# pengpeng-yu/FastPCC

Hardware: NVIDIA B200
Metric: encode+decode Mpts/s (higher is better)
Workload: dtype int8

## Files before the change

fastpcc_b200/csrc/igemm_tc.cu:

```cuda
#include <cuda.h>
#include <cuda_bf16.h>
#include <cuda_fp16.h>

#include <map>
#include <mutex>
#include <tuple>

#include "common.cuh"
#include "epi_nt.cuh"

namespace fpcc {

constexpr int TC_M = 128;
constexpr int TC_KB = 128;
constexpr int TC_MAX_KVOL = 32;

__device__ __forceinline__ uint32_t smem_u32(const void *p) { return (uint32_t)__cvta_generic_to_shared(p); }

__device__ __forceinline__ void mbar_init(uint64_t *bar, uint32_t count) {
    asm volatile("mbarrier.init.shared::cta.b64 [%0], %1;" ::"r"(smem_u32(bar)), "r"(count));
}
__device__ __forceinline__ void mbar_arrive(uint64_t *bar) {
    asm volatile("mbarrier.arrive.shared::cta.b64 _, [%0];" ::"r"(smem_u32(bar)) : "memory");
}
// ... 32 lines not shown
    asm volatile("mov.u32 %0, %%cluster_ctarank;" : "=r"(r));
    return r;
}
__device__ __forceinline__ uint32_t mapa_u32(uint32_t local_smem_addr, uint32_t rank) {
    uint32_t a;
    asm volatile("mapa.shared::cluster.u32 %0, %1, %2;" : "=r"(a) : "r"(local_smem_addr), "r"(rank));
    return a;
}
__device__ __forceinline__ void cluster_sync_all() {
    asm volatile("barrier.cluster.arrive.release.aligned;" ::: "memory");
    asm volatile("barrier.cluster.wait.acquire.aligned;" ::: "memory");
}
__device__ __forceinline__ void mbar_wait_cluster(uint64_t *bar, uint32_t parity) {
    asm volatile(
        "{\n\t"
        ".reg .pred p;\n\t"
        "WAITC_LOOP:\n\t"
        "mbarrier.try_wait.parity.acquire.cluster.shared::cta.b64 p, [%0], %1, %2;\n\t"
        "@p bra.uni WAITC_DONE;\n\t"
        "bra.uni WAITC_LOOP;\n\t"
        "WAITC_DONE:\n\t"
        "}" ::"r"(smem_u32(bar)), "r"(parity), "r"(0x989680u) : "memory");
}
__device__ __forceinline__ void tma_load_2d_mc(uint32_t dst, const CUtensorMap *map, uint64_t *bar, int c0, int c1, uint16_t cta_mask) {
    asm volatile(
        "cp.async.bulk.tensor.2d.shared::cluster.global.mbarrier::complete_tx::bytes.multicast::cluster [%0], [%1, {%3, %4}], [%2], %5;"
        ::"r"(dst), "l"(map), "r"(smem_u32(bar)), "r"(c0), "r"(c1), "h"(cta_mask) : "memory");
}
__device__ __forceinline__ void umma_commit_mc(uint64_t *bar, uint16_t cta_mask) {
    asm volatile("tcgen05.commit.cta_group::1.mbarrier::arrive::one.shared::cluster.multicast::cluster.b64 [%0], %1;"
                 ::"r"(smem_u32(bar)), "h"(cta_mask) : "memory");
}
__device__ __forceinline__ void cp_async16(uint32_t dst, const void *src, uint32_t src_bytes) {
    asm volatile("cp.async.cg.shared.global [%0], [%1], 16, %2;" ::"r"(dst), "l"(src), "r"(src_bytes) : "memory");
}
__device__ __forceinline__ void cp_async_commit() { asm volatile("cp.async.commit_group;" ::: "memory"); }
template <int N>
__device__ __forceinline__ void cp_async_wait() { asm volatile("cp.async.wait_group %0;" ::"n"(N) : "memory"); }
__device__ __forceinline__ void fence_proxy_async() { asm volatile("fence.proxy.async.shared::cta;" ::: "memory"); }
__device__ __forceinline__ void tc_fence_before() { asm volatile("tcgen05.fence::before_thread_sync;" ::: "memory"); }
__device__ __forceinline__ void tc_fence_after() { asm volatile("tcgen05.fence::after_thread_sync;" ::: "memory"); }

__device__ __forceinline__ void tma_load_2d(uint32_t dst, const CUtensorMap *map, uint64_t *bar, int c0, int c1) {
    asm volatile(
        "cp.async.bulk.tensor.2d.shared::cluster.global.mbarrier::complete_tx::bytes [%0], [%1, {%3, %4}], [%2];"
        ::"r"(dst), "l"(map), "r"(smem_u32(bar)), "r"(c0), "r"(c1) : "memory");
}

__device__ __forceinline__ uint64_t umma_desc_sw128(uint32_t smem_addr) {
    uint64_t d = 0;
    d |= (uint64_t)((smem_addr & 0x3FFFFu) >> 4);
    d |= (uint64_t)(1024u >> 4) << 32;
    d |= (uint64_t)1 << 46;
    d |= (uint64_t)2 << 61;
    return d;
}
__device__ __forceinline__ uint32_t umma_idesc_i8(int n) {
    return (2u << 4) | (1u << 7) | (1u << 10) | ((uint32_t)(n >> 3) << 17) | ((uint32_t)(TC_M >> 4) << 24);
}
__device__ __forceinline__ uint32_t umma_idesc_f16(int n, int bf16) {
    return (1u << 4) | ((uint32_t)bf16 << 7) | ((uint32_t)bf16 << 10) | ((uint32_t)(n >> 3) << 17) | ((uint32_t)(TC_M >> 4) << 24);
}
__device__ __forceinline__ void umma_f16(uint32_t tmem_d, uint64_t adesc, uint64_t bdesc, uint32_t idesc, uint32_t accumulate) {
    asm volatile(
        "{\n\t"
        ".reg .pred p;\n\t"
        "setp.ne.b32 p, %4, 0;\n\t"
        "tcgen05.mma.cta_group::1.kind::f16 [%0], %1, %2, %3, p;\n\t"
        "}" ::"r"(tmem_d), "l"(adesc), "l"(bdesc), "r"(idesc), "r"(accumulate) : "memory");
}
__device__ __forceinline__ void umma_i8(uint32_t tmem_d, uint64_t adesc, uint64_t bdesc, uint32_t idesc, uint32_t accumulate) {
    asm volatile(
        "{\n\t"
        ".reg .pred p;\n\t"
        "setp.ne.b32 p, %4, 0;\n\t"
        "tcgen05.mma.cta_group::1.kind::i8 [%0], %1, %2, %3, p;\n\t"
        "}" ::"r"(tmem_d), "l"(adesc), "l"(bdesc), "r"(idesc), "r"(accumulate) : "memory");
}
__device__ __forceinline__ void umma_commit(uint64_t *bar) {
    asm volatile("tcgen05.commit.cta_group::1.mbarrier::arrive::one.shared::cluster.b64 [%0];" ::"r"(smem_u32(bar)) : "memory");
}
__device__ __forceinline__ void tmem_ld16(uint32_t taddr, uint32_t (&r)[16]) {
    asm volatile(
        "tcgen05.ld.sync.aligned.32x32b.x16.b32 "
        "{%0, %1, %2, %3, %4, %5, %6, %7, %8, %9, %10, %11, %12, %13, %14, %15}, [%16];"
        : "=r"(r[0]), "=r"(r[1]), "=r"(r[2]), "=r"(r[3]), "=r"(r[4]), "=r"(r[5]), "=r"(r[6]), "=r"(r[7]), "=r"(r[8]),
          "=r"(r[9]), "=r"(r[10]), "=r"(r[11]), "=r"(r[12]), "=r"(r[13]), "=r"(r[14]), "=r"(r[15])
        : "r"(taddr));
    asm volatile("tcgen05.wait::ld.sync.aligned;" ::: "memory");
}

#ifdef FPCC_TC_TRACE
__device__ unsigned long long g_trace[4096][8];
__device__ __forceinline__ void trace_stamp(int j, int slot) {
    if (blockIdx.x == 0 && j < 4096) {
        unsigned long long t;
        asm volatile("mov.u64 %0, %%globaltimer;" : "=l"(t));
        g_trace[j][slot] = t;
    }
}
#define TRACE(j, slot) trace_stamp((j), (slot))
#else
#define TRACE(j, slot)
#endif

struct TcArgs {
    const int8_t *A;
    int K;
    int N;
    int n_tile;
    int tmem_cols;
    const int32_t *nbr;
    int64_t ld;
    int n_out, kvol;
    const int32_t *row_perm;
    const int32_t *in_idx, *out_idx, *offsets;
    int n_groups, n_pairs, bias_per_group;
};

constexpr int EC = 16;

template <int WORDS>
__device__ __forceinline__ void store_words(char *optr, const uint32_t (&w)[WORDS], int nbytes) {
#pragma unroll
    for (int t = 0; t < WORDS / 4; ++t)
        if (t * 16 < nbytes) reinterpret_cast<uint4 *>(optr)[t] = make_uint4(w[4 * t], w[4 * t + 1], w[4 * t + 2], w[4 * t + 3]);
// ... 698 lines not shown
                if (fe.out_type == 0) ((__half *)optr)[q] = __float2half_rn(o[q]);
                else if (fe.out_type == 1) ((__nv_bfloat16 *)optr)[q] = __float2bfloat16_rn(o[q]);
                else ((float *)optr)[q] = o[q];
            }
        }
    }
}

constexpr int EPI_WARPS_CONV = 12, EPI_WARPS_PAIRS = 16;
#ifndef FPCC_PAIRS_PRODUCER_WARPS
#define FPCC_PAIRS_PRODUCER_WARPS 4
#endif
template <int MODE>
constexpr int prod_warps() { return MODE == 1 ? FPCC_PAIRS_PRODUCER_WARPS : 4; }
static_assert(FPCC_PAIRS_PRODUCER_WARPS == 4 || FPCC_PAIRS_PRODUCER_WARPS == 2, "producer warps: 2 or 4");

struct PMeta {
    uint32_t kmask;
    int32_t group, begin, end;
};

template <int STAGES>
struct PSmem {
    static size_t bytes(int n_tile, int rows_k) {
        return 1024 + (size_t)STAGES * (TC_M * TC_KB + (size_t)n_tile * TC_KB) + 2 * (size_t)rows_k * TC_M * 4 +
               (size_t)n_tile * 20 + 512;
    }
};

__device__ __forceinline__ void pairs_tile_lookup(const TcArgs &a, int tile_m, PMeta *m) {
    int g = 0, begin = tile_m * TC_M, end = a.n_pairs;
    if (a.offsets) {
        int t = tile_m;
        begin = end = -1;
        for (g = 0; g < a.n_groups; ++g) {
            int lo = a.offsets[g], hi = a.offsets[g + 1];
            int nt = (hi - lo + TC_M - 1) / TC_M;
            if (t < nt) { begin = lo + t * TC_M; end = hi; break; }
            t -= nt;
        }
    }
    m->group = g < a.n_groups ? g : a.n_groups - 1; m->begin = begin; m->end = end;
}

enum { OK_I8 = 0, OK_I16 = 1, OK_I32 = 2, OK_POST2 = 3 };

template <int MODE, int STAGES, int KIND, int EW, int OUTK, bool CL2>
__global__ void __launch_bounds__((EW + prod_warps<MODE>() + 2) * 32, 1) igemm_tc_persistent(TcArgs a, const __grid_constant__ CUtensorMap tmap_w,
                                                                    EpiParams ep, FEpi fe, void *__restrict__ out, int tiles_m,
                                                                    int tiles_n) {
    constexpr int PW = prod_warps<MODE>(), PT = PW * 32;
    constexpr int P_EPI_WARPS = EW, P_PROD_WARP0 = EW, P_TMA_WARP = EW + PW, P_MMA_WARP = EW + PW + 1, P_THREADS = (EW + PW + 2) * 32;
    extern __shared__ uint8_t smem_raw[];
    uint8_t *smem = (uint8_t *)(((uintptr_t)smem_raw + 1023) & ~(uintptr_t)1023);
    const int b_bytes = a.n_tile * TC_KB;
    constexpr int a_bytes = TC_M * TC_KB;
    uint8_t *sA = smem;
    uint8_t *sB = smem + STAGES * a_bytes;
    const int rows_k = MODE == 0 ? a.kvol : 2;
    int32_t *rows_s = (int32_t *)(sB + (size_t)STAGES * b_bytes);
    int4 *chan4_s = (int4 *)(rows_s + 2 * rows_k * TC_M);
    int2 *chan_s = (int2 *)chan4_s;
    int32_t *thr_s = (int32_t *)(chan4_s + a.n_tile);
    uint64_t *bars = (uint64_t *)(thr_s + a.n_tile);
    uint64_t *full = bars, *empty = bars + STAGES;
    uint64_t *meta_full = bars + 2 * STAGES, *tmem_full = meta_full + 2, *tmem_empty = tmem_full + 2;
    uint64_t *xchg = tmem_empty + 2;
    uint64_t *meta_empty = xchg + 2;
    PMeta *meta = (PMeta *)(meta_empty + 2);
    uint32_t *tmem_ptr = (uint32_t *)(meta + 2);
    uint32_t *lean_off = tmem_ptr + 1;
    uint32_t *peer_kmask = lean_off + 1;
    uint32_t *nt_flags = peer_kmask + 2;
    const uint32_t cl_rank = CL2 ? cluster_ctarank() : 0u;
    const int p0 = CL2 ? (int)(blockIdx.x >> 1) : (int)blockIdx.x;
    const int p_step = CL2 ? (int)(gridDim.x >> 1) : (int)gridDim.x;

    const int tid = threadIdx.x, warp = tid >> 5, lane = tid & 31;
    const int n_chunks = (a.K + TC_KB - 1) / TC_KB;
    const int total_tiles = tiles_m * tiles_n;
    const int p_end = CL2 ? (total_tiles + 1) / 2 : total_tiles;
#define FPCC_TILE_OF(p) (CL2 ? 2 * (p) + (int)cl_rank : (p))

    if (warp == P_MMA_WARP && lane == 0) {
        for (int s = 0; s < STAGES; ++s) {
            mbar_init(&full[s], PT + 1);
            mbar_init(&empty[s], CL2 ? 2 : 1);
        }
        for (int b = 0; b < 2; ++b) {
            mbar_init(&meta_full[b], PT);
            mbar_init(&tmem_full[b], 1);
            mbar_init(&tmem_empty[b], P_EPI_WARPS);
            mbar_init(&xchg[b], 1);
            mbar_init(&meta_empty[b], P_EPI_WARPS + 2);
        }
        asm volatile("fence.mbarrier_init.release.cluster;" ::: "memory");
    }
    if (warp == P_TMA_WARP && lane == 0) asm volatile("prefetch.tensormap [%0];" ::"l"(&tmap_w) : "memory");
    if (warp == P_MMA_WARP) {
        asm volatile("tcgen05.alloc.cta_group::1.sync.aligned.shared::cta.b32 [%0], %1;" ::"r"(smem_u32(tmem_ptr)), "r"((uint32_t)(2 * a.tmem_cols)) : "memory");
        asm volatile("tcgen05.relinquish_alloc_permit.cta_group::1.sync.aligned;" ::: "memory");
    }
    const bool chan_static = tiles_n == 1 && !(MODE == 1 && a.bias_per_group);
    const int64_t zp_all = KIND == 0 ? ep.zp[0] : 0;
    int64_t vmax = 0;
    const int sgn_mode = KIND == 0 ? lean_mode(ep, zp_all, (int64_t)a.K * (MODE == 0 ? a.kvol : 1), ep.row_bias_bound, &vmax) : SGN_NONE;
    if (tid >= 32 && tid < 48) nt_flags[tid - 32] = 0u;
    if (tid == 0) {
        *lean_off = sgn_mode != SGN_NONE ? 0u : 1u;
        thr_s[0] = (1 << 24) - 1; thr_s[1] = 0;
        if (KIND == 0 && ep.post_mul) {
            const Post2 p2 = load_post2(ep);
            int64_t t2 = 0;
            if (p2.mul) { const int64_t nz = -p2.zp, m = (int64_t)p2.mul; t2 = nz >= 0 ? (nz + m - 1) / m : -((-nz) / m); }
            const int64_t c02 = p2.zp + (p2.shift > 0 ? (int64_t)1 << (p2.shift - 1) : 0);
            thr_s[4] = (int32_t)p2.mul;
            thr_s[5] = (int32_t)(t2 > 2147483647ll ? 2147483647ll : (t2 < -2147483648ll ? -2147483648ll : t2));
            thr_s[6] = p2.slope; thr_s[7] = p2.shift >= 32 ? p2.shift - 32 : 0;
            thr_s[8] = (int32_t)(uint32_t)c02; thr_s[9] = (int32_t)(uint32_t)((uint64_t)c02 >> 32);
            thr_s[10] = (p2.shift >= 32 && !tie_possible(p2.mul, p2.zp, p2.shift, (int64_t)1 << 31)) ? 1 : 0;
        }
    }
    __syncthreads();
    const bool nt_on = FPCC_NT_SMEM && KIND == 0 && OUTK == OK_I8 && sgn_mode != SGN_NONE;
    const int64_t abound = (int64_t)a.K * (MODE == 0 ? a.kvol : 1) * 16384 + (ep.row_bias ? (int64_t)ep.row_bias_bound : 0);
    if (chan_static)
        for (int cb = warp * 32; cb < a.n_tile; cb += P_THREADS) {
            const int c = cb + lane;
            const bool valid = c < a.n_tile;
            if (KIND == 0) {
                const int32_t b = c < a.N && ep.bias ? ep.bias[c] : 0;
                const uint32_t mu = c < a.N ? ep.mul[ep.mul_is_scalar ? 0 : c] : 0u;
                bool ok = true;
                if (valid) {
                    ok = stage_channel(b, mu, zp_all, ep.shift, ep.out_type, vmax, &chan4_s[c]);
                    if (!ok && sgn_mode != SGN_NONE) atomicOr(lean_off, 1u);
                }
                stage_nt_chunks(nt_on, valid, ok, c, b, mu, zp_all, ep.shift, abound, nt_flags);
            } else if (valid) {
                chan_s[c] = make_int2(c < a.N && fe.bias ? __float_as_int(fe.bias[c]) : 0, 0);
            }
        }
    tc_fence_before();
    __syncthreads();
    tc_fence_after();
    if (CL2) cluster_sync_all();
    const uint32_t tmem_base = *tmem_ptr;

    if (warp >= P_PROD_WARP0 && warp < P_PROD_WARP0 + PW) {
        const int r = tid - P_PROD_WARP0 * 32;
        int it = 0;
        int j = 0;
        constexpr int PRE = 27;
        int32_t nv[PRE];
        const bool pre = MODE == 0 && a.kvol <= PRE;
        auto fetch = [&](int t) {
            const int m = (t / tiles_n) * TC_M + r;
            const bool ok = t < total_tiles && m < a.n_out;
#pragma unroll
            for (int u = 0; u < PRE; ++u) nv[u] = (ok && u < a.kvol) ? __ldg(&a.nbr[(int64_t)u * a.ld + m]) : 0;
        };
        if (pre) fetch(FPCC_TILE_OF(p0));
        for (int p = p0; p < p_end; p += p_step, ++j) {
            const int tile = FPCC_TILE_OF(p);
            const int slot = j & 1;
            const int tile_m = tile / tiles_n;
            int32_t *rows = rows_s + slot * rows_k * TC_M;
            if (r == 0) TRACE(j, 0);
            mbar_wait(&meta_empty[slot], ((j >> 1) & 1) ^ 1);
// ... 19 lines not shown
                    }
                }
                mine = __reduce_or_sync(0xffffffffu, mine);
                if (lane == 0 && mine) atomicOr(&meta[slot].kmask, mine);
            } else {
                if (r == 0) { pairs_tile_lookup(a, tile_m, &meta[slot]); }
                asm volatile("bar.sync 1, %0;" ::"n"(PT) : "memory");
#if FPCC_PAIRS_PRODUCER_WARPS == 4
                const int p = meta[slot].begin + r;
                const bool ok = meta[slot].begin >= 0 && p < meta[slot].end;
                rows[r] = ok ? (a.in_idx ? __ldg(&a.in_idx[p]) : p) : -1;
                rows[TC_M + r] = ok ? (a.out_idx ? __ldg(&a.out_idx[p]) : p) : -1;
#else
#pragma unroll
                for (int rr = r; rr < TC_M; rr += PT) {
                    const int p = meta[slot].begin + rr;
                    const bool ok = meta[slot].begin >= 0 && p < meta[slot].end;
                    rows[rr] = ok ? (a.in_idx ? __ldg(&a.in_idx[p]) : p) : -1;
                    rows[TC_M + rr] = ok ? (a.out_idx ? __ldg(&a.out_idx[p]) : p) : -1;
                }
#endif
                if (r == 0) meta[slot].kmask = meta[slot].begin >= 0 && meta[slot].begin < meta[slot].end ? 1u : 0u;
            }
            if (CL2) {
                asm volatile("bar.sync 1, %0;" ::"n"(PT) : "memory");
                if (r == 0) {
                    const uint32_t own = *(volatile uint32_t *)&meta[slot].kmask;
                    const uint32_t peer = cl_rank ^ 1u;
                    asm volatile("st.shared::cluster.u32 [%0], %1;" ::"r"(mapa_u32(smem_u32(&peer_kmask[slot]), peer)), "r"(own) : "memory");
                    asm volatile("mbarrier.arrive.release.cluster.shared::cluster.b64 _, [%0];" ::"r"(mapa_u32(smem_u32(&xchg[slot]), peer)) : "memory");
                    mbar_wait_cluster(&xchg[slot], (j >> 1) & 1);
                    meta[slot].kmask = own | *(volatile uint32_t *)&peer_kmask[slot];
                }
            }
            __threadfence_block();
            mbar_arrive(&meta_full[slot]);
            mbar_wait(&meta_full[slot], (j >> 1) & 1);
            uint32_t rem = meta[slot].kmask;
            const int total = __popc(rem) * n_chunks;
            int k = 0, kc = n_chunks - 1;
            if (r == 0) TRACE(j, 2);
            for (int i = 0; i < total; ++i, ++it) {
                if (++kc == n_chunks) { kc = 0; k = __ffs(rem) - 1; rem &= rem - 1; }
                const int stage = it % STAGES;
                mbar_wait(&empty[stage], ((it / STAGES) & 1) ^ 1);
#if FPCC_PAIRS_PRODUCER_WARPS == 4
                const int base = (r & ~31) + (lane >> 3) * 8;
// ... 36 lines not shown
                }
#endif
                asm volatile("cp.async.mbarrier.arrive.noinc.shared::cta.b64 [%0];" ::"r"(smem_u32(&full[stage])) : "memory");
            }
        }
    } else if (warp == P_TMA_WARP) {
        if (lane == 0) {
            int it = 0, j = 0;
            for (int p = p0; p < p_end; p += p_step, ++j) {
                const int tile = FPCC_TILE_OF(p);
                const int slot = j & 1;
                const int n0 = (tile % tiles_n) * a.n_tile;
                mbar_wait(&meta_full[slot], (j >> 1) & 1);
                uint32_t rem = meta[slot].kmask;
                const int total = __popc(rem) * n_chunks;
                const int group = MODE == 1 ? meta[slot].group : 0;
                mbar_arrive(&meta_empty[slot]);
                int k = 0, kc = n_chunks - 1;
                for (int i = 0; i < total; ++i, ++it) {
                    if (++kc == n_chunks) { kc = 0; k = __ffs(rem) - 1; rem &= rem - 1; }
                    const int stage = it % STAGES;
                    mbar_wait(&empty[stage], ((it / STAGES) & 1) ^ 1);
                    mbar_expect_tx(&full[stage], (uint32_t)b_bytes);
                    const int wrow = (MODE == 0 ? k : group) * a.N + n0;
                    if (CL2) {
                        const int half = a.n_tile >> 1;
                        tma_load_2d_mc(smem_u32(sB + (size_t)stage * b_bytes + (size_t)cl_rank * half * TC_KB), &tmap_w, &full[stage],
                                       kc * TC_KB, wrow + (int)cl_rank * half, (uint16_t)3);
                    } else {
                        tma_load_2d(smem_u32(sB + (size_t)stage * b_bytes), &tmap_w, &full[stage], kc * TC_KB, wrow);
                    }
                }
            }
        }
    } else if (warp == P_MMA_WARP) {
        if (lane == 0) {
            const uint32_t idesc = KIND == 0 ? umma_idesc_i8(a.n_tile) : umma_idesc_f16(a.n_tile, KIND == 2);
            int it = 0, j = 0;
            for (int p = p0; p < p_end; p += p_step, ++j) {
                const int slot = j & 1;
                mbar_wait(&meta_full[slot], (j >> 1) & 1);
                const int total = __popc(meta[slot].kmask) * n_chunks;
                mbar_arrive(&meta_empty[slot]);
                mbar_wait(&tmem_empty[slot], ((j >> 1) & 1) ^ 1);
                tc_fence_after();
                const uint32_t tacc = tmem_base + (uint32_t)(slot * a.tmem_cols);
                for (int i = 0; i < total; ++i, ++it) {
                    const int stage = it % STAGES;
                    mbar_wait(&full[stage], (it / STAGES) & 1);
                    if (i == 0) TRACE(j, 3);
                    fence_proxy_async();
                    tc_fence_after();
                    const uint64_t ad = umma_desc_sw128(smem_u32(sA + stage * a_bytes));
                    const uint64_t bd = umma_desc_sw128(smem_u32(sB + (size_t)stage * b_bytes));
                    {
#pragma unroll
                        for (int q = 0; q < TC_KB / 32; ++q) {
                            if (KIND == 0) umma_i8(tacc, ad + 2 * q, bd + 2 * q, idesc, (uint32_t)(i > 0 || q > 0));
                            else umma_f16(tacc, ad + 2 * q, bd + 2 * q, idesc, (uint32_t)(i > 0 || q > 0));
                        }
                    }
                    if (CL2) umma_commit_mc(&empty[stage], (uint16_t)3);
                    else umma_commit(&empty[stage]);
                }
                TRACE(j, 4);
                if (total > 0) umma_commit(&tmem_full[slot]);
                else mbar_arrive(&tmem_full[slot]);
            }
        }
    } else if (warp < P_EPI_WARPS) {
        const int quarter = warp & 3, group = warp >> 2;
        const int r = quarter * 32 + lane;
        const bool has_slope = KIND == 0 && ep.slope != nullptr, has_post = KIND == 0 && ep.post_slope != nullptr;
        const int32_t slope = has_slope ? ep.slope[0] : 0, post = has_post ? ep.post_slope[0] : 0;
        const int64_t zp = KIND == 0 ? ep.zp[0] : 0;
        const int shift = ep.shift;
        const int cols_grp = (((a.n_tile + P_EPI_WARPS / 4 - 1) / (P_EPI_WARPS / 4) + EC - 1) / EC) * EC;
        const int c_begin = min(a.n_tile, group * cols_grp), c_end = min(a.n_tile, c_begin + cols_grp);
        const bool out_al = ((uintptr_t)out & 15) == 0 && (ep.out_ld & 15) == 0;
        LeanU lu;
        {
            const int64_t c0v = zp + (shift > 0 ? (int64_t)1 << (shift - 1) : 0);
            lu.slope = slope; lu.post = post; lu.shift = shift; { const uint32_t ka = smem_u32(thr_s); int32_t k_lo, k_hi; asm volatile("ld.shared.v2.s32 {%0, %1}, [%2];" : "=r"(k_lo), "=r"(k_hi) : "r"(ka)); lu.k24 = pack64((uint32_t)k_lo, (uint32_t)k_hi); }
            lu.c0_lo = (uint32_t)c0v; lu.c0_hi = (uint32_t)((uint64_t)c0v >> 32);
            lu.ovf_add = shift > 0 && shift <= 31 ? 1u << (shift - 1) : 0u;
            lu.ovf_lim = shift <= 31 ? (1u << shift) - 1u : 0xffffffffu;
        }
        lu.post2_addr = smem_u32(thr_s + 4);
        lu.nt_addr = smem_u32(nt_flags);
        const bool post2_on = KIND == 0 && OUTK == OK_POST2;
// ... 133 lines not shown
                EpiCtx cx;
                cx.chan4 = chan4_s + c0;
                cx.slope = slope; cx.post = post; cx.zp = zp; cx.shift = shift;
                cx.half = shift > 0 ? (int64_t)1 << (shift - 1) : 0; cx.sgn = shift > 0;
                cx.row_bias = ep.row_bias ? ep.row_bias + (int64_t)__ldg(&ep.row_idx[m]) * a.N + nb : nullptr;
                cx.residual = ep.residual ? ep.residual + m * a.N + nb : nullptr;
                cx.has_post = has_post;
                cx.nvalid = min(EC, a.N - nb);
                void *optr = (ep.out_type == FPCC_OUT_I8 || post2_on) ? (void *)((char *)out + m * (ep.out_ld > 0 ? (int64_t)ep.out_ld : (int64_t)a.N) + nb)
                                                                      : (void *)((char *)out + (m * a.N + nb) * (ep.out_type == FPCC_OUT_I16 ? 2 : 4));
                const bool vec = out_al && (a.N & 15) == 0;
                const bool rb = ep.row_bias != nullptr;
                Post2 p2;
                p2.on = false; p2.dual = false;
                if (post2_on || (OUTK == OK_I32 && ep.aux_out)) p2 = load_post2(ep);
                cx.aux = p2.dual ? ep.aux_out + m * a.N + nb : nullptr;
                if (OUTK == OK_I8) epi_dispatch<FPCC_OUT_I8>(acc, cx, optr, vec, has_slope, rb, p2);
                else if (OUTK == OK_I32 || OUTK == OK_POST2) epi_dispatch<FPCC_OUT_I32>(acc, cx, optr, vec, has_slope, rb, p2);
                else epi_dispatch<FPCC_OUT_I16>(acc, cx, optr, vec, has_slope, rb, p2);
            }
            tc_fence_before();
            __syncwarp();
            if (tid == 0) TRACE(j, 6);
            if (lane == 0) mbar_arrive(&tmem_empty[slot]);
        }
    }
    tc_fence_before();
    __syncthreads();
    if (CL2) cluster_sync_all();
    if (warp == P_MMA_WARP) {
        asm volatile("tcgen05.dealloc.cta_group::1.sync.aligned.b32 %0, %1;" ::"r"(tmem_base), "r"((uint32_t)(2 * a.tmem_cols)) : "memory");
    }
#undef FPCC_TILE_OF
}

__global__ void __launch_bounds__(128, 1) mma_i8_peak_kernel(int iters, int n) {
    extern __shared__ uint8_t smem_raw[];
    uint8_t *smem = (uint8_t *)(((uintptr_t)smem_raw + 1023) & ~(uintptr_t)1023);
    __shared__ uint64_t done;
    __shared__ uint32_t tmem_ptr;
    const int warp = threadIdx.x >> 5, lane = threadIdx.x & 31;
    for (int i = threadIdx.x; i < (TC_M * TC_KB + 256 * TC_KB) / 4; i += blockDim.x) ((uint32_t *)smem)[i] = 0x01010101u;
    if (threadIdx.x == 0) {
        mbar_init(&done, 1);
        asm volatile("fence.mbarrier_init.release.cluster;" ::: "memory");
    }
    if (warp == 0) {
        asm volatile("tcgen05.alloc.cta_group::1.sync.aligned.shared::cta.b32 [%0], %1;" ::"r"(smem_u32(&tmem_ptr)), "r"(256u) : "memory");
        asm volatile("tcgen05.relinquish_alloc_permit.cta_group::1.sync.aligned;" ::: "memory");
    }
    fence_proxy_async();
    tc_fence_before();
    __syncthreads();
    tc_fence_after();
    const uint32_t tmem_base = tmem_ptr;
// ... 56 lines not shown
    CUresult r = fn(&m, CU_TENSOR_MAP_DATA_TYPE_UINT8, 2, (void *)w, dims, strides, box, estr, CU_TENSOR_MAP_INTERLEAVE_NONE,
                    CU_TENSOR_MAP_SWIZZLE_128B, CU_TENSOR_MAP_L2_PROMOTION_L2_256B, CU_TENSOR_MAP_FLOAT_OOB_FILL_NONE);
    FPCC_REQUIRE(r == CUDA_SUCCESS, "cuTensorMapEncodeTiled failed with CUresult %d (rows %lld, K %d, box %d)", (int)r, (long long)rows, K, box_rows);
    if (cache.size() > 4096) cache.clear();
    cache[key] = m;
    *out = m;
    return FPCC_OK;
}

static bool tc_shape_ok(const void *A, const void *W, int K, int N) {
    return K >= 32 && K % 16 == 0 && N >= 16 && (((uintptr_t)A | (uintptr_t)W) & 15) == 0;
}

static int pick_tile(int N, int *n_tile, int *tmem_cols) {
    int nt = N >= 256 ? 256 : ((N + 15) / 16) * 16;
    int cols = 32;
    while (cols < nt) cols <<= 1;
    *n_tile = nt;
    *tmem_cols = cols;
    return (N + nt - 1) / nt;
}

constexpr size_t TC_SMEM_MAX = 227 * 1024;
template <int MODE, int STAGES, int KIND, int OUTK>
static int launch_outk(const TcArgs &a, const CUtensorMap &tmap, const EpiParams &ep, const FEpi &fe, void *out, int tiles_m,
                       int n_blocks_n, int grid, size_t smem, bool cl2, cudaStream_t s) {
#ifndef FPCC_CONV2_EW
#define FPCC_CONV2_EW 8
#endif
#ifndef FPCC_LIN32_EW
#define FPCC_LIN32_EW 8
#endif
#ifndef FPCC_LINP2_EW
#define FPCC_LINP2_EW 8
#endif
#ifndef FPCC_CONV1_EW
#define FPCC_CONV1_EW EPI_WARPS_CONV
#endif
#ifndef FPCC_LIN8_EW
#define FPCC_LIN8_EW EPI_WARPS_PAIRS
#endif
    constexpr int EW = KIND != 0 ? (MODE == 0 ? EPI_WARPS_CONV : EPI_WARPS_PAIRS)
                       : MODE == 0 ? ((OUTK == OK_I32 || OUTK == OK_POST2) ? FPCC_CONV2_EW : FPCC_CONV1_EW)
                                   : (OUTK == OK_I32 ? FPCC_LIN32_EW : (OUTK == OK_POST2 ? FPCC_LINP2_EW : FPCC_LIN8_EW));
    constexpr int OK = KIND == 0 ? OUTK : OK_I8;
    constexpr int THREADS = (EW + prod_warps<MODE>() + 2) * 32;
    if (MODE == 0 && KIND == 0 && cl2) {
        auto kern = igemm_tc_persistent<MODE, STAGES, KIND, EW, OK, (MODE == 0 && KIND == 0)>;
        static bool configured = false;
        if (!configured) {
            FPCC_CUDA(cudaFuncSetAttribute(kern, cudaFuncAttributeMaxDynamicSharedMemorySize, (int)TC_SMEM_MAX));
            configured = true;
        }
        cudaLaunchConfig_t cfg = {};
        cfg.gridDim = dim3((unsigned)grid); cfg.blockDim = dim3(THREADS); cfg.dynamicSmemBytes = smem; cfg.stream = s;
        cudaLaunchAttribute attr[1];
        attr[0].id = cudaLaunchAttributeClusterDimension;
        attr[0].val.clusterDim.x = 2; attr[0].val.clusterDim.y = 1; attr[0].val.clusterDim.z = 1;
        cfg.attrs = attr; cfg.numAttrs = 1;
        FPCC_CUDA(cudaLaunchKernelEx(&cfg, kern, a, tmap, ep, fe, out, tiles_m, n_blocks_n));
        return FPCC_OK;
    }
    auto kern = igemm_tc_persistent<MODE, STAGES, KIND, EW, OK, false>;
    static bool configured = false;
    if (!configured) {
        FPCC_CUDA(cudaFuncSetAttribute(kern, cudaFuncAttributeMaxDynamicSharedMemorySize, (int)TC_SMEM_MAX));
        configured = true;
    }
    kern<<<grid, THREADS, smem, s>>>(a, tmap, ep, fe, out, tiles_m, n_blocks_n);
    FPCC_LAUNCH_CHECK();
    return FPCC_OK;
}

template <int MODE, int STAGES, int KIND>
static int launch_stages(const TcArgs &a, const CUtensorMap &tmap, const EpiParams &ep, const FEpi &fe, void *out, int tiles_m,
                         int n_blocks_n, int grid, int rows_k, bool cl2, cudaStream_t s) {
    size_t smem = PSmem<STAGES>::bytes(a.n_tile, rows_k);
    FPCC_REQUIRE(smem <= TC_SMEM_MAX, "igemm_tc: %zu bytes of shared memory exceed the 227 KB limit", smem);
    if (KIND != 0) return launch_outk<MODE, STAGES, KIND, OK_I8>(a, tmap, ep, fe, out, tiles_m, n_blocks_n, grid, smem, cl2, s);
    if (ep.post_mul && !ep.aux_out) return launch_outk<MODE, STAGES, KIND, OK_POST2>(a, tmap, ep, fe, out, tiles_m, n_blocks_n, grid, smem, cl2, s);
    if (ep.out_type == FPCC_OUT_I8) return launch_outk<MODE, STAGES, KIND, OK_I8>(a, tmap, ep, fe, out, tiles_m, n_blocks_n, grid, smem, cl2, s);
    if (ep.out_type == FPCC_OUT_I32) return launch_outk<MODE, STAGES, KIND, OK_I32>(a, tmap, ep, fe, out, tiles_m, n_blocks_n, grid, smem, cl2, s);
    return launch_outk<MODE, STAGES, KIND, OK_I16>(a, tmap, ep, fe, out, tiles_m, n_blocks_n, grid, smem, cl2, s);
}

static int g_cl2_mode = -1;
static bool cl2_enabled() {
    if (g_cl2_mode < 0) {
        const char *e = getenv("FPCC_CL2");
        g_cl2_mode = (e && e[0] == '1') ? 1 : 0;
    }
    return g_cl2_mode == 1;
}

template <int MODE, int KIND>
static int launch_tc(TcArgs &a, const void *W, int64_t w_rows, int tiles_m, const EpiParams &ep, const FEpi &fe, void *out,
                     cudaStream_t s) {
    int n_blocks_n = pick_tile(a.N, &a.n_tile, &a.tmem_cols);
    const int rows_k = MODE == 0 ? a.kvol : 2;
    int total = tiles_m * n_blocks_n;
    int sms = g_sm_budget > 0 && g_sm_budget < sm_count() ? g_sm_budget : sm_count();
    const bool cl2 = MODE == 0 && KIND == 0 && n_blocks_n == 1 && (a.n_tile % 16) == 0 && total >= 4 && sms >= 2 && cl2_enabled();
    CUtensorMap tmap;
    int rc = weight_tensor_map((const int8_t *)W, w_rows, a.K, cl2 ? a.n_tile / 2 : a.n_tile, &tmap);
    if (rc) return rc;
    int grid = total < sms ? total : sms;
    if (cl2) {
        const int pairs = (total + 1) / 2, clusters = sms / 2;
        grid = 2 * (pairs < clusters ? pairs : clusters);
    }
    static const bool force3 = [] { const char *e = getenv("FPCC_STAGES"); return e && e[0] == '3'; }();
    if (!force3 && PSmem<4>::bytes(a.n_tile, rows_k) <= TC_SMEM_MAX)
        return launch_stages<MODE, 4, KIND>(a, tmap, ep, fe, out, tiles_m, n_blocks_n, grid, rows_k, cl2, s);
    return launch_stages<MODE, 3, KIND>(a, tmap, ep, fe, out, tiles_m, n_blocks_n, grid, rows_k, cl2, s);
}

int launch_conv_tc(const int8_t *feats, int n_in, int c_in, const int8_t *weight, int kvol, int c_out, const int32_t *nbr,
                   int64_t ld, int n_out, const int32_t *row_perm, const EpiParams &ep, void *out, cudaStream_t s) {
    (void)n_in;
    if (!tc_shape_ok(feats, weight, c_in, c_out) || kvol > TC_MAX_KVOL) return FPCC_ERR_UNSUPPORTED;
    TcArgs a = {};
    a.A = feats; a.K = c_in; a.N = c_out;
    a.nbr = nbr; a.ld = ld; a.n_out = n_out; a.kvol = kvol; a.row_perm = row_perm;
    FEpi fe = {};
    return launch_tc<0, 0>(a, weight, (int64_t)kvol * c_out, ceil_div(n_out, TC_M), ep, fe, out, s);
}

int launch_pairs_tc(const PairArgs &p, const EpiParams &ep, void *out, int max_tiles, cudaStream_t s) {
    (void)max_tiles;
    if (p.raw != 0 || !tc_shape_ok(p.A, p.W, p.K, p.N)) return FPCC_ERR_UNSUPPORTED;
    TcArgs a = {};
    a.A = p.A; a.K = p.K; a.N = p.N;
    a.in_idx = p.in_idx; a.out_idx = p.out_idx; a.offsets = p.offsets;
    a.n_groups = p.n_groups; a.n_pairs = p.n_pairs; a.bias_per_group = p.bias_per_group;
    int tiles = ceil_div(p.n_pairs, TC_M) + (p.offsets ? p.n_groups : 0);
    FEpi fe = {};
    return launch_tc<1, 0>(a, p.W, (int64_t)p.n_groups * p.N, tiles, ep, fe, out, s);
// ... 259 lines not shown
    cudaStream_t s = (cudaStream_t)stream;
    size_t smem = 1024 + TC_M * TC_KB + 256 * TC_KB;
    FPCC_CUDA(cudaFuncSetAttribute(mma_i8_peak_kernel, cudaFuncAttributeMaxDynamicSharedMemorySize, (int)smem));
    cudaEvent_t e0, e1;
    FPCC_CUDA(cudaEventCreate(&e0));
    FPCC_CUDA(cudaEventCreate(&e1));
    int sms = sm_count();
    mma_i8_peak_kernel<<<sms, 128, smem, s>>>(iters / 8 + 1, n);
    FPCC_CUDA(cudaEventRecord(e0, s));
    mma_i8_peak_kernel<<<sms, 128, smem, s>>>(iters, n);
    FPCC_CUDA(cudaEventRecord(e1, s));
    FPCC_CUDA(cudaEventSynchronize(e1));
    float ms = 0;
    FPCC_CUDA(cudaEventElapsedTime(&ms, e0, e1));
    cudaEventDestroy(e0);
    cudaEventDestroy(e1);
    *tops_out = 2.0 * TC_M * n * 32.0 * 4.0 * iters * sms / (ms * 1e-3) / 1e12;
    return FPCC_OK;
}

#ifdef FPCC_TC_TRACE
extern "C" int fpcc_trace_read(unsigned long long *host, int n) {
    FPCC_CUDA(cudaDeviceSynchronize());
    FPCC_CUDA(cudaMemcpyFromSymbol(host, fpcc::g_trace, sizeof(unsigned long long) * 8 * (size_t)n));
    return FPCC_OK;
}
#endif

extern "C" int fpcc_gemm_engine(int k, int n, int kvol, int has_zp_comp) {
    return fpcc::tc_enabled() && !has_zp_comp && k >= 32 && k % 16 == 0 && n >= 16 && kvol <= fpcc::TC_MAX_KVOL;
}

extern "C" int fpcc_set_sm_budget(int sms) {
    fpcc::g_sm_budget = sms > 0 ? sms : 0;
    return FPCC_OK;
}

extern "C" int fpcc_set_tc_mode(int mode) {
    fpcc::g_tc_mode = mode ? 1 : 0;
    return FPCC_OK;
}
```

Baseline: 24.90.

## Use 2-CTA paired tcgen05 MMA for sparse conv tiles by default

Replaces the opt-in 2-CTA cluster mode, which multicast weights via TMA, with a true cta_group::2 UMMA path. Each CTA loads half of the weight tile and the leader issues M=256 MMAs spanning both CTAs. Paired TMEM alloc, remote mbarrier arrivals and a 6-stage pipeline support this, and it is enabled by default for conv with int8, int32 or post2 outputs. The aim is to halve per-CTA weight smem traffic and make the tensor cores more efficient. In exchange it adds cross-CTA synchronisation, and the two CTAs now run their tiles in lockstep, so the slower tile sets the pace.

```diff
diff --git a/fastpcc_b200/csrc/igemm_tc.cu b/fastpcc_b200/csrc/igemm_tc.cu
--- a/fastpcc_b200/csrc/igemm_tc.cu
+++ b/fastpcc_b200/csrc/igemm_tc.cu
@@ -78,14 +78,35 @@
         "WAITC_DONE:\n\t"
         "}" ::"r"(smem_u32(bar)), "r"(parity), "r"(0x989680u) : "memory");
 }
-__device__ __forceinline__ void tma_load_2d_mc(uint32_t dst, const CUtensorMap *map, uint64_t *bar, int c0, int c1, uint16_t cta_mask) {
+__device__ __forceinline__ void mbar_arrive_remote(uint64_t *bar, uint32_t rank) {
+    asm volatile("mbarrier.arrive.release.cluster.shared::cluster.b64 _, [%0];" ::"r"(mapa_u32(smem_u32(bar), rank)) : "memory");
+}
+__device__ __forceinline__ void umma_i8_pair(uint32_t tmem_d, uint64_t adesc, uint64_t bdesc, uint32_t idesc, uint32_t accumulate) {
     asm volatile(
-        "cp.async.bulk.tensor.2d.shared::cluster.global.mbarrier::complete_tx::bytes.multicast::cluster [%0], [%1, {%3, %4}], [%2], %5;"
-        ::"r"(dst), "l"(map), "r"(smem_u32(bar)), "r"(c0), "r"(c1), "h"(cta_mask) : "memory");
-}
-__device__ __forceinline__ void umma_commit_mc(uint64_t *bar, uint16_t cta_mask) {
-    asm volatile("tcgen05.commit.cta_group::1.mbarrier::arrive::one.shared::cluster.multicast::cluster.b64 [%0], %1;"
-                 ::"r"(smem_u32(bar)), "h"(cta_mask) : "memory");
+        "{\n\t"
+        ".reg .pred p;\n\t"
+        "setp.ne.b32 p, %4, 0;\n\t"
+        "tcgen05.mma.cta_group::2.kind::i8 [%0], %1, %2, %3, p;\n\t"
+        "}" ::"r"(tmem_d), "l"(adesc), "l"(bdesc), "r"(idesc), "r"(accumulate) : "memory");
+}
+__device__ __forceinline__ void umma_commit_pair(uint64_t *bar) {
+    asm volatile("tcgen05.commit.cta_group::2.mbarrier::arrive::one.shared::cluster.multicast::cluster.b64 [%0], %1;"
+                 ::"r"(smem_u32(bar)), "h"((uint16_t)3) : "memory");
+}
+template <bool PAIR>
+__device__ __forceinline__ void tmem_alloc(uint32_t *dst, uint32_t cols) {
+    if (PAIR) {
+        asm volatile("tcgen05.alloc.cta_group::2.sync.aligned.shared::cta.b32 [%0], %1;" ::"r"(smem_u32(dst)), "r"(cols) : "memory");
+        asm volatile("tcgen05.relinquish_alloc_permit.cta_group::2.sync.aligned;" ::: "memory");
+    } else {
+        asm volatile("tcgen05.alloc.cta_group::1.sync.aligned.shared::cta.b32 [%0], %1;" ::"r"(smem_u32(dst)), "r"(cols) : "memory");
+        asm volatile("tcgen05.relinquish_alloc_permit.cta_group::1.sync.aligned;" ::: "memory");
+    }
+}
+template <bool PAIR>
+__device__ __forceinline__ void tmem_dealloc(uint32_t base, uint32_t cols) {
+    if (PAIR) asm volatile("tcgen05.dealloc.cta_group::2.sync.aligned.b32 %0, %1;" ::"r"(base), "r"(cols) : "memory");
+    else asm volatile("tcgen05.dealloc.cta_group::1.sync.aligned.b32 %0, %1;" ::"r"(base), "r"(cols) : "memory");
 }
 __device__ __forceinline__ void cp_async16(uint32_t dst, const void *src, uint32_t src_bytes) {
     asm volatile("cp.async.cg.shared.global [%0], [%1], 16, %2;" ::"r"(dst), "l"(src), "r"(src_bytes) : "memory");
@@ -111,8 +132,8 @@
     d |= (uint64_t)2 << 61;
     return d;
 }
-__device__ __forceinline__ uint32_t umma_idesc_i8(int n) {
-    return (2u << 4) | (1u << 7) | (1u << 10) | ((uint32_t)(n >> 3) << 17) | ((uint32_t)(TC_M >> 4) << 24);
+__device__ __forceinline__ uint32_t umma_idesc_i8(int n, int m = TC_M) {
+    return (2u << 4) | (1u << 7) | (1u << 10) | ((uint32_t)(n >> 3) << 17) | ((uint32_t)(m >> 4) << 24);
 }
 __device__ __forceinline__ uint32_t umma_idesc_f16(int n, int bf16) {
     return (1u << 4) | ((uint32_t)bf16 << 7) | ((uint32_t)bf16 << 10) | ((uint32_t)(n >> 3) << 17) | ((uint32_t)(TC_M >> 4) << 24);
@@ -147,17 +168,26 @@
 }
 
 #ifdef FPCC_TC_TRACE
-__device__ unsigned long long g_trace[4096][8];
+constexpr int TRACE_SLOTS = 16;
+__device__ unsigned long long g_trace[4096][TRACE_SLOTS];
+__device__ __forceinline__ unsigned long long trace_now() {
+    unsigned long long t;
+    asm volatile("mov.u64 %0, %%globaltimer;" : "=l"(t));
+    return t;
+}
 __device__ __forceinline__ void trace_stamp(int j, int slot) {
-    if (blockIdx.x == 0 && j < 4096) {
-        unsigned long long t;
-        asm volatile("mov.u64 %0, %%globaltimer;" : "=l"(t));
-        g_trace[j][slot] = t;
-    }
+    if (blockIdx.x == 0 && j < 4096) g_trace[j][slot] = trace_now();
+}
+__device__ __forceinline__ void trace_add(int j, int slot, unsigned long long v, bool first) {
+    if (blockIdx.x == 0 && j < 4096) g_trace[j][slot] = (first ? 0ull : g_trace[j][slot]) + v;
 }
 #define TRACE(j, slot) trace_stamp((j), (slot))
+#define TRACE_NOW() trace_now()
+#define TRACE_ADD(j, slot, v, first) trace_add((j), (slot), (v), (first))
 #else
 #define TRACE(j, slot)
+#define TRACE_NOW() 0ull
+#define TRACE_ADD(j, slot, v, first)
 #endif
 
 struct TcArgs {
@@ -902,8 +932,8 @@
 
 template <int STAGES>
 struct PSmem {
-    static size_t bytes(int n_tile, int rows_k) {
-        return 1024 + (size_t)STAGES * (TC_M * TC_KB + (size_t)n_tile * TC_KB) + 2 * (size_t)rows_k * TC_M * 4 +
+    static size_t bytes(int n_tile, int rows_k, bool pair = false) {
+        return 1024 + (size_t)STAGES * (TC_M * TC_KB + (size_t)(pair ? n_tile / 2 : n_tile) * TC_KB) + 2 * (size_t)rows_k * TC_M * 4 +
                (size_t)n_tile * 20 + 512;
     }
 };
@@ -925,7 +955,7 @@
 
 enum { OK_I8 = 0, OK_I16 = 1, OK_I32 = 2, OK_POST2 = 3 };
 
-template <int MODE, int STAGES, int KIND, int EW, int OUTK, bool CL2>
+template <int MODE, int STAGES, int KIND, int EW, int OUTK, bool PAIR>
 __global__ void __launch_bounds__((EW + prod_warps<MODE>() + 2) * 32, 1) igemm_tc_persistent(TcArgs a, const __grid_constant__ CUtensorMap tmap_w,
                                                                     EpiParams ep, FEpi fe, void *__restrict__ out, int tiles_m,
                                                                     int tiles_n) {
@@ -933,7 +963,7 @@
     constexpr int P_EPI_WARPS = EW, P_PROD_WARP0 = EW, P_TMA_WARP = EW + PW, P_MMA_WARP = EW + PW + 1, P_THREADS = (EW + PW + 2) * 32;
     extern __shared__ uint8_t smem_raw[];
     uint8_t *smem = (uint8_t *)(((uintptr_t)smem_raw + 1023) & ~(uintptr_t)1023);
-    const int b_bytes = a.n_tile * TC_KB;
+    const int b_bytes = (PAIR ? a.n_tile / 2 : a.n_tile) * TC_KB;
     constexpr int a_bytes = TC_M * TC_KB;
     uint8_t *sA = smem;
     uint8_t *sB = smem + STAGES * a_bytes;
@@ -952,35 +982,33 @@
     uint32_t *lean_off = tmem_ptr + 1;
     uint32_t *peer_kmask = lean_off + 1;
     uint32_t *nt_flags = peer_kmask + 2;
-    const uint32_t cl_rank = CL2 ? cluster_ctarank() : 0u;
-    const int p0 = CL2 ? (int)(blockIdx.x >> 1) : (int)blockIdx.x;
-    const int p_step = CL2 ? (int)(gridDim.x >> 1) : (int)gridDim.x;
+    const uint32_t cl_rank = PAIR ? cluster_ctarank() : 0u;
+    const bool leader = cl_rank == 0u;
+    const int p0 = PAIR ? (int)(blockIdx.x >> 1) : (int)blockIdx.x;
+    const int p_step = PAIR ? (int)(gridDim.x >> 1) : (int)gridDim.x;
 
     const int tid = threadIdx.x, warp = tid >> 5, lane = tid & 31;
     const int n_chunks = (a.K + TC_KB - 1) / TC_KB;
     const int total_tiles = tiles_m * tiles_n;
-    const int p_end = CL2 ? (total_tiles + 1) / 2 : total_tiles;
-#define FPCC_TILE_OF(p) (CL2 ? 2 * (p) + (int)cl_rank : (p))
+    const int p_end = PAIR ? (total_tiles + 1) / 2 : total_tiles;
+#define FPCC_TILE_OF(p) (PAIR ? 2 * (p) + (int)cl_rank : (p))
 
     if (warp == P_MMA_WARP && lane == 0) {
         for (int s = 0; s < STAGES; ++s) {
-            mbar_init(&full[s], PT + 1);
-            mbar_init(&empty[s], CL2 ? 2 : 1);
+            mbar_init(&full[s], PT + 1 + (PAIR && leader ? 1 : 0));
+            mbar_init(&empty[s], 1);
         }
         for (int b = 0; b < 2; ++b) {
             mbar_init(&meta_full[b], PT);
             mbar_init(&tmem_full[b], 1);
-            mbar_init(&tmem_empty[b], P_EPI_WARPS);
+            mbar_init(&tmem_empty[b], PAIR ? 2 * P_EPI_WARPS : P_EPI_WARPS);
             mbar_init(&xchg[b], 1);
             mbar_init(&meta_empty[b], P_EPI_WARPS + 2);
         }
         asm volatile("fence.mbarrier_init.release.cluster;" ::: "memory");
     }
     if (warp == P_TMA_WARP && lane == 0) asm volatile("prefetch.tensormap [%0];" ::"l"(&tmap_w) : "memory");
-    if (warp == P_MMA_WARP) {
-        asm volatile("tcgen05.alloc.cta_group::1.sync.aligned.shared::cta.b32 [%0], %1;" ::"r"(smem_u32(tmem_ptr)), "r"((uint32_t)(2 * a.tmem_cols)) : "memory");
-        asm volatile("tcgen05.relinquish_alloc_permit.cta_group::1.sync.aligned;" ::: "memory");
-    }
+    if (warp == P_MMA_WARP) tmem_alloc<PAIR>(tmem_ptr, (uint32_t)(2 * a.tmem_cols));
     const bool chan_static = tiles_n == 1 && !(MODE == 1 && a.bias_per_group);
     const int64_t zp_all = KIND == 0 ? ep.zp[0] : 0;
     int64_t vmax = 0;
@@ -1024,7 +1052,7 @@
     tc_fence_before();
     __syncthreads();
     tc_fence_after();
-    if (CL2) cluster_sync_all();
+    if (PAIR) cluster_sync_all();
     const uint32_t tmem_base = *tmem_ptr;
 
     if (warp >= P_PROD_WARP0 && warp < P_PROD_WARP0 + PW) {
@@ -1090,7 +1118,7 @@
 #endif
                 if (r == 0) meta[slot].kmask = meta[slot].begin >= 0 && meta[slot].begin < meta[slot].end ? 1u : 0u;
             }
-            if (CL2) {
+            if (PAIR) {
                 asm volatile("bar.sync 1, %0;" ::"n"(PT) : "memory");
                 if (r == 0) {
                     const uint32_t own = *(volatile uint32_t *)&meta[slot].kmask;
@@ -1173,32 +1201,53 @@
                     const int stage = it % STAGES;
                     mbar_wait(&empty[stage], ((it / STAGES) & 1) ^ 1);
                     mbar_expect_tx(&full[stage], (uint32_t)b_bytes);
-                    const int wrow = (MODE == 0 ? k : group) * a.N + n0;
-                    if (CL2) {
-                        const int half = a.n_tile >> 1;
-                        tma_load_2d_mc(smem_u32(sB + (size_t)stage * b_bytes + (size_t)cl_rank * half * TC_KB), &tmap_w, &full[stage],
-                                       kc * TC_KB, wrow + (int)cl_rank * half, (uint16_t)3);
-                    } else {
-                        tma_load_2d(smem_u32(sB + (size_t)stage * b_bytes), &tmap_w, &full[stage], kc * TC_KB, wrow);
-                    }
-                }
-            }
-        }
-    } else if (warp == P_MMA_WARP) {
+                    const int wrow = (MODE == 0 ? k : group) * a.N + n0 + (int)cl_rank * (a.n_tile >> 1);
+                    tma_load_2d(smem_u32(sB + (size_t)stage * b_bytes), &tmap_w, &full[stage], kc * TC_KB, wrow);
+                }
+            }
+            if (PAIR) {
+                for (int i = 0; i < STAGES; ++i, ++it) mbar_wait(&empty[it % STAGES], ((it / STAGES) & 1) ^ 1);
+            }
+        }
+    } else if (warp == P_MMA_WARP && PAIR && !leader) {
         if (lane == 0) {
-            const uint32_t idesc = KIND == 0 ? umma_idesc_i8(a.n_tile) : umma_idesc_f16(a.n_tile, KIND == 2);
             int it = 0, j = 0;
             for (int p = p0; p < p_end; p += p_step, ++j) {
                 const int slot = j & 1;
                 mbar_wait(&meta_full[slot], (j >> 1) & 1);
                 const int total = __popc(meta[slot].kmask) * n_chunks;
                 mbar_arrive(&meta_empty[slot]);
-                mbar_wait(&tmem_empty[slot], ((j >> 1) & 1) ^ 1);
+                for (int i = 0; i < total; ++i, ++it) {
+                    const int stage = it % STAGES;
+                    mbar_wait(&full[stage], (it / STAGES) & 1);
+                    fence_proxy_async();
+                    mbar_arrive_remote(&full[stage], 0u);
+                }
+            }
+        }
+    } else if (warp == P_MMA_WARP) {
+        if (lane == 0) {
+            const uint32_t idesc = KIND == 0 ? umma_idesc_i8(a.n_tile, PAIR ? 2 * TC_M : TC_M) : umma_idesc_f16(a.n_tile, KIND == 2);
+            int it = 0, j = 0;
+            for (int p = p0; p < p_end; p += p_step, ++j) {
+                const int slot = j & 1;
+                mbar_wait(&meta_full[slot], (j >> 1) & 1);
+                const int total = __popc(meta[slot].kmask) * n_chunks;
+                mbar_arrive(&meta_empty[slot]);
+                TRACE(j, 7);
+                if (PAIR) mbar_wait_cluster(&tmem_empty[slot], ((j >> 1) & 1) ^ 1);
+                else mbar_wait(&tmem_empty[slot], ((j >> 1) & 1) ^ 1);
+                TRACE(j, 8);
                 tc_fence_after();
                 const uint32_t tacc = tmem_base + (uint32_t)(slot * a.tmem_cols);
                 for (int i = 0; i < total; ++i, ++it) {
                     const int stage = it % STAGES;
-                    mbar_wait(&full[stage], (it / STAGES) & 1);
+                    const unsigned long long tw = TRACE_NOW();
+                    if (PAIR) mbar_wait_cluster(&full[stage], (it / STAGES) & 1);
+                    else mbar_wait(&full[stage], (it / STAGES) & 1);
+                    TRACE_ADD(j, 9, TRACE_NOW() - tw, i == 0);
+                    TRACE_ADD(j, 10, 1ull, i == 0);
+                    (void)tw;
                     if (i == 0) TRACE(j, 3);
                     fence_proxy_async();
                     tc_fence_after();
@@ -1207,16 +1256,22 @@
                     {
 #pragma unroll
                         for (int q = 0; q < TC_KB / 32; ++q) {
-                            if (KIND == 0) umma_i8(tacc, ad + 2 * q, bd + 2 * q, idesc, (uint32_t)(i > 0 || q > 0));
+                            if (PAIR) umma_i8_pair(tacc, ad + 2 * q, bd + 2 * q, idesc, (uint32_t)(i > 0 || q > 0));
+                            else if (KIND == 0) umma_i8(tacc, ad + 2 * q, bd + 2 * q, idesc, (uint32_t)(i > 0 || q > 0));
                             else umma_f16(tacc, ad + 2 * q, bd + 2 * q, idesc, (uint32_t)(i > 0 || q > 0));
                         }
                     }
-                    if (CL2) umma_commit_mc(&empty[stage], (uint16_t)3);
+                    if (PAIR) umma_commit_pair(&empty[stage]);
                     else umma_commit(&empty[stage]);
                 }
                 TRACE(j, 4);
-                if (total > 0) umma_commit(&tmem_full[slot]);
-                else mbar_arrive(&tmem_full[slot]);
+                if (PAIR) {
+                    if (total > 0) umma_commit_pair(&tmem_full[slot]);
+                    else { mbar_arrive(&tmem_full[slot]); mbar_arrive_remote(&tmem_full[slot], 1u); }
+                } else {
+                    if (total > 0) umma_commit(&tmem_full[slot]);
+                    else mbar_arrive(&tmem_full[slot]);
+                }
             }
         }
     } else if (warp < P_EPI_WARPS) {
@@ -1396,15 +1451,16 @@
             tc_fence_before();
             __syncwarp();
             if (tid == 0) TRACE(j, 6);
-            if (lane == 0) mbar_arrive(&tmem_empty[slot]);
+            if (lane == 0) {
+                if (PAIR) mbar_arrive_remote(&tmem_empty[slot], 0u);
+                else mbar_arrive(&tmem_empty[slot]);
+            }
         }
     }
     tc_fence_before();
     __syncthreads();
-    if (CL2) cluster_sync_all();
-    if (warp == P_MMA_WARP) {
-        asm volatile("tcgen05.dealloc.cta_group::1.sync.aligned.b32 %0, %1;" ::"r"(tmem_base), "r"((uint32_t)(2 * a.tmem_cols)) : "memory");
-    }
+    if (PAIR) cluster_sync_all();
+    if (warp == P_MMA_WARP) tmem_dealloc<PAIR>(tmem_base, (uint32_t)(2 * a.tmem_cols));
 #undef FPCC_TILE_OF
 }
 
@@ -1507,9 +1563,14 @@
 }
 
 constexpr size_t TC_SMEM_MAX = 227 * 1024;
-template <int MODE, int STAGES, int KIND, int OUTK>
+constexpr int PAIR_STAGES = 6;
+#ifndef FPCC_CONV_PAIR
+#define FPCC_CONV_PAIR ((1 << OK_I8) | (1 << OK_I32) | (1 << OK_POST2))
+#endif
+
+template <int MODE, int STAGES, int KIND, int OUTK, bool PAIR>
 static int launch_outk(const TcArgs &a, const CUtensorMap &tmap, const EpiParams &ep, const FEpi &fe, void *out, int tiles_m,
-                       int n_blocks_n, int grid, size_t smem, bool cl2, cudaStream_t s) {
+                       int n_blocks_n, int grid, size_t smem, cudaStream_t s) {
 #ifndef FPCC_CONV2_EW
 #define FPCC_CONV2_EW 8
 #endif
@@ -1530,13 +1591,13 @@
                                    : (OUTK == OK_I32 ? FPCC_LIN32_EW : (OUTK == OK_POST2 ? FPCC_LINP2_EW : FPCC_LIN8_EW));
     constexpr int OK = KIND == 0 ? OUTK : OK_I8;
     constexpr int THREADS = (EW + prod_warps<MODE>() + 2) * 32;
-    if (MODE == 0 && KIND == 0 && cl2) {
-        auto kern = igemm_tc_persistent<MODE, STAGES, KIND, EW, OK, (MODE == 0 && KIND == 0)>;
-        static bool configured = false;
-        if (!configured) {
-            FPCC_CUDA(cudaFuncSetAttribute(kern, cudaFuncAttributeMaxDynamicSharedMemorySize, (int)TC_SMEM_MAX));
-            configured = true;
-        }
+    auto kern = igemm_tc_persistent<MODE, STAGES, KIND, EW, OK, PAIR>;
+    static bool configured = false;
+    if (!configured) {
+        FPCC_CUDA(cudaFuncSetAttribute(kern, cudaFuncAttributeMaxDynamicSharedMemorySize, (int)TC_SMEM_MAX));
+        configured = true;
+    }
+    if constexpr (PAIR) {
         cudaLaunchConfig_t cfg = {};
         cfg.gridDim = dim3((unsigned)grid); cfg.blockDim = dim3(THREADS); cfg.dynamicSmemBytes = smem; cfg.stream = s;
         cudaLaunchAttribute attr[1];
@@ -1546,36 +1607,40 @@
         FPCC_CUDA(cudaLaunchKernelEx(&cfg, kern, a, tmap, ep, fe, out, tiles_m, n_blocks_n));
         return FPCC_OK;
     }
-    auto kern = igemm_tc_persistent<MODE, STAGES, KIND, EW, OK, false>;
-    static bool configured = false;
-    if (!configured) {
-        FPCC_CUDA(cudaFuncSetAttribute(kern, cudaFuncAttributeMaxDynamicSharedMemorySize, (int)TC_SMEM_MAX));
-        configured = true;
-    }
     kern<<<grid, THREADS, smem, s>>>(a, tmap, ep, fe, out, tiles_m, n_blocks_n);
     FPCC_LAUNCH_CHECK();
     return FPCC_OK;
 }
 
+static int outk_of(const EpiParams &ep) {
+    if (ep.post_mul && !ep.aux_out) return OK_POST2;
+    if (ep.out_type == FPCC_OUT_I8) return OK_I8;
+    if (ep.out_type == FPCC_OUT_I32) return OK_I32;
+    return OK_I16;
+}
+
 template <int MODE, int STAGES, int KIND>
 static int launch_stages(const TcArgs &a, const CUtensorMap &tmap, const EpiParams &ep, const FEpi &fe, void *out, int tiles_m,
-                         int n_blocks_n, int grid, int rows_k, bool cl2, cudaStream_t s) {
+                         int n_blocks_n, int grid, int rows_k, cudaStream_t s) {
     size_t smem = PSmem<STAGES>::bytes(a.n_tile, rows_k);
     FPCC_REQUIRE(smem <= TC_SMEM_MAX, "igemm_tc: %zu bytes of shared memory exceed the 227 KB limit", smem);
-    if (KIND != 0) return launch_outk<MODE, STAGES, KIND, OK_I8>(a, tmap, ep, fe, out, tiles_m, n_blocks_n, grid, smem, cl2, s);
-    if (ep.post_mul && !ep.aux_out) return launch_outk<MODE, STAGES, KIND, OK_POST2>(a, tmap, ep, fe, out, tiles_m, n_blocks_n, grid, smem, cl2, s);
-    if (ep.out_type == FPCC_OUT_I8) return launch_outk<MODE, STAGES, KIND, OK_I8>(a, tmap, ep, fe, out, tiles_m, n_blocks_n, grid, smem, cl2, s);
-    if (ep.out_type == FPCC_OUT_I32) return launch_outk<MODE, STAGES, KIND, OK_I32>(a, tmap, ep, fe, out, tiles_m, n_blocks_n, grid, smem, cl2, s);
-    return launch_outk<MODE, STAGES, KIND, OK_I16>(a, tmap, ep, fe, out, tiles_m, n_blocks_n, grid, smem, cl2, s);
-}
-
-static int g_cl2_mode = -1;
-static bool cl2_enabled() {
-    if (g_cl2_mode < 0) {
-        const char *e = getenv("FPCC_CL2");
-        g_cl2_mode = (e && e[0] == '1') ? 1 : 0;
-    }
-    return g_cl2_mode == 1;
+    if (KIND != 0) return launch_outk<MODE, STAGES, KIND, OK_I8, false>(a, tmap, ep, fe, out, tiles_m, n_blocks_n, grid, smem, s);
+    switch (outk_of(ep)) {
+        case OK_POST2: return launch_outk<MODE, STAGES, KIND, OK_POST2, false>(a, tmap, ep, fe, out, tiles_m, n_blocks_n, grid, smem, s);
+        case OK_I8: return launch_outk<MODE, STAGES, KIND, OK_I8, false>(a, tmap, ep, fe, out, tiles_m, n_blocks_n, grid, smem, s);
+        case OK_I32: return launch_outk<MODE, STAGES, KIND, OK_I32, false>(a, tmap, ep, fe, out, tiles_m, n_blocks_n, grid, smem, s);
+        default: return launch_outk<MODE, STAGES, KIND, OK_I16, false>(a, tmap, ep, fe, out, tiles_m, n_blocks_n, grid, smem, s);
+    }
+}
+
+template <int OUTK>
+static int launch_pair(const TcArgs &a, const CUtensorMap &tmap, const EpiParams &ep, void *out, int tiles_m, int grid, cudaStream_t s) {
+    if constexpr (((FPCC_CONV_PAIR >> OUTK) & 1) != 0) {
+        const FEpi fe = {};
+        return launch_outk<0, PAIR_STAGES, 0, OUTK, true>(a, tmap, ep, fe, out, tiles_m, 1, grid,
+                                                          PSmem<PAIR_STAGES>::bytes(a.n_tile, a.kvol, true), s);
+    }
+    return FPCC_ERR_UNSUPPORTED;
 }
 
 template <int MODE, int KIND>
@@ -1585,19 +1650,24 @@
     const int rows_k = MODE == 0 ? a.kvol : 2;
     int total = tiles_m * n_blocks_n;
     int sms = g_sm_budget > 0 && g_sm_budget < sm_count() ? g_sm_budget : sm_count();
-    const bool cl2 = MODE == 0 && KIND == 0 && n_blocks_n == 1 && (a.n_tile % 16) == 0 && total >= 4 && sms >= 2 && cl2_enabled();
+    const int outk = KIND == 0 ? outk_of(ep) : OK_I8;
+    const bool pair = MODE == 0 && KIND == 0 && n_blocks_n == 1 && (a.n_tile % 32) == 0 && sms >= 2 && ((FPCC_CONV_PAIR >> outk) & 1) &&
+                      PSmem<PAIR_STAGES>::bytes(a.n_tile, rows_k, true) <= TC_SMEM_MAX;
     CUtensorMap tmap;
-    int rc = weight_tensor_map((const int8_t *)W, w_rows, a.K, cl2 ? a.n_tile / 2 : a.n_tile, &tmap);
+    int rc = weight_tensor_map((const int8_t *)W, w_rows, a.K, pair ? a.n_tile / 2 : a.n_tile, &tmap);
     if (rc) return rc;
+    if (pair) {
+        const int pairs = (total + 1) / 2, clusters = sms / 2;
+        const int grid = 2 * (pairs < clusters ? pairs : clusters);
+        if (outk == OK_I8) return launch_pair<OK_I8>(a, tmap, ep, out, tiles_m, grid, s);
+        if (outk == OK_I32) return launch_pair<OK_I32>(a, tmap, ep, out, tiles_m, grid, s);
+        return launch_pair<OK_POST2>(a, tmap, ep, out, tiles_m, grid, s);
+    }
     int grid = total < sms ? total : sms;
-    if (cl2) {
-        const int pairs = (total + 1) / 2, clusters = sms / 2;
-        grid = 2 * (pairs < clusters ? pairs : clusters);
-    }
     static const bool force3 = [] { const char *e = getenv("FPCC_STAGES"); return e && e[0] == '3'; }();
     if (!force3 && PSmem<4>::bytes(a.n_tile, rows_k) <= TC_SMEM_MAX)
-        return launch_stages<MODE, 4, KIND>(a, tmap, ep, fe, out, tiles_m, n_blocks_n, grid, rows_k, cl2, s);
-    return launch_stages<MODE, 3, KIND>(a, tmap, ep, fe, out, tiles_m, n_blocks_n, grid, rows_k, cl2, s);
+        return launch_stages<MODE, 4, KIND>(a, tmap, ep, fe, out, tiles_m, n_blocks_n, grid, rows_k, s);
+    return launch_stages<MODE, 3, KIND>(a, tmap, ep, fe, out, tiles_m, n_blocks_n, grid, rows_k, s);
 }
 
 int launch_conv_tc(const int8_t *feats, int n_in, int c_in, const int8_t *weight, int kvol, int c_out, const int32_t *nbr,
@@ -1903,7 +1973,7 @@
 #ifdef FPCC_TC_TRACE
 extern "C" int fpcc_trace_read(unsigned long long *host, int n) {
     FPCC_CUDA(cudaDeviceSynchronize());
-    FPCC_CUDA(cudaMemcpyFromSymbol(host, fpcc::g_trace, sizeof(unsigned long long) * 8 * (size_t)n));
+    FPCC_CUDA(cudaMemcpyFromSymbol(host, fpcc::g_trace, sizeof(unsigned long long) * fpcc::TRACE_SLOTS * (size_t)n));
     return FPCC_OK;
 }
 #endif
```

After: 23.70 (median of 6 runs). 0.952x the previous value.
